# qianyizh/ElasticReconstruction

Measured on AMD Instinct MI355X. Metric: depth frames/sec into 512^3 TSDF (640x480), higher is better.
Workload: dtype f32; 1 GPU; configs[1]; frames_per_gpu=91800, volume_units_touched=122, warp=True, inputs=hbm_resident, parallelism=single GPU

## Files before the change

### elasticreconstruction_amd/_ffi.py

```python
import ctypes as C
import os

_HERE = os.path.dirname(os.path.abspath(__file__))
LIB_PATH = os.environ.get("ER_HIP_LIB") or os.path.join(_HERE, "liber_hip.so")

SYMBOLS = [
    "er_last_error", "er_device_count", "er_abi_version", "er_request_hw_queues", "er_host_alloc", "er_host_free", "er_host_copy_h2d", "er_device_alloc", "er_device_free", "er_device_copy_d2h",
    "er_tsdf_create", "er_tsdf_destroy", "er_tsdf_set_stream", "er_tsdf_synchronize",
    "er_tsdf_wait_event", "er_tsdf_reset", "er_tsdf_status", "er_tsdf_set_unit_shard", "er_unit_owner",
    "er_tsdf_scale_depth", "er_tsdf_reproject", "er_tsdf_integrate", "er_tsdf_integrate_frames", "er_tsdf_prepass_trace", "er_tsdf_set_zbuf_epoch",
    "er_tsdf_unit_count", "er_tsdf_unit_keys", "er_tsdf_read_unit", "er_tsdf_sum_weight",
    "er_tsdf_extract_world", "er_tsdf_extract_surface", "er_tsdf_extract_oriented", "er_tsdf_extract_mesh", "er_mc_table", "er_tsdf_extract_mesh_indexed", "er_mesh_components", "er_tsdf_extract_mesh_cleaned", "er_tsdf_import_world", "er_raycast_params_default", "er_tsdf_raycast", "er_tsdf_raycast_batch", "er_tsdf_export_weighted", "er_tsdf_import_weighted",
    "er_tsdf_export_raw", "er_tsdf_import_raw",
    "er_tsdf_color_enable", "er_tsdf_read_unit_color", "er_tsdf_write_unit_color", "er_tsdf_color_frames", "er_tsdf_reproject_color", "er_tsdf_sample_colors",
    "er_tsdf_band_sizes", "er_tsdf_export_band", "er_tsdf_merge_band", "er_tsdf_import_band", "er_tsdf_drop_units",
    "er_tsdf_set_profiling", "er_tsdf_get_profile", "er_tsdf_set_timeline", "er_tsdf_get_timeline",
    "er_comm_unique_id", "er_comm_create", "er_comm_create_local", "er_comm_create_loopback", "er_comm_destroy", "er_comm_rank", "er_comm_world",
    "er_tsdf_allreduce", "er_comm_merge_stats", "er_comm_merge_stats_owner", "er_frame_block",
    "er_cloud_create", "er_cloud_create_batch", "er_cloud_create_from_tsdf", "er_cloud_destroy", "er_cloud_size",
    "er_icp_count_inliers", "er_icp_align", "er_icp_align_trace", "er_find_correspondence",
    "er_icp_count_inliers_batch", "er_icp_align_batch", "er_find_correspondence_batch", "er_icp_release_workspaces", "er_registration_batch", "er_ransac_fitness_batch", "er_ransac_inliers",
    "er_features_create", "er_features_destroy", "er_features_size", "er_feature_knn", "er_ransac_hypotheses", "er_ransac_params_default", "er_ransac_align", "er_ransac_align_batch",
    "er_odom_params_default", "er_odom_create", "er_odom_destroy", "er_odom_align_pairs", "er_odom_track", "er_frame_to_model_align", "er_frames_to_models_align", "er_odom_linearize", "er_odom_read_maps", "er_odom_tables",
    "er_cloud_read", "er_cloud_voxel_grid", "er_cloud_estimate_normals", "er_fpfh_estimate", "er_features_dim", "er_features_read",
    "er_frag_params_default", "er_frag_create", "er_frag_destroy", "er_frag_lane_bytes", "er_frag_build", "er_frag_count", "er_frag_read",
# ... 72 lines not shown
    L.er_tsdf_create.argtypes = [C.c_int, C.c_int, fp, C.c_int, C.c_int, C.POINTER(vp)]
    L.er_tsdf_destroy.argtypes = [vp]
    L.er_tsdf_set_stream.argtypes = [vp, vp]
    L.er_tsdf_synchronize.argtypes = [vp]
    L.er_tsdf_wait_event.argtypes = [vp, vp]
    L.er_tsdf_reset.argtypes = [vp]
    L.er_tsdf_status.argtypes = [vp, ip, C.POINTER(C.c_long)]
    L.er_tsdf_set_unit_shard.argtypes = [vp, C.c_int, C.c_int]
    L.er_unit_owner.argtypes = [C.c_int, C.c_int]
    L.er_tsdf_scale_depth.argtypes = [vp, vp, vp]
    L.er_tsdf_reproject.argtypes = [vp, vp, vp, C.c_int, C.c_float, vp, vp]
    L.er_tsdf_integrate.argtypes = [vp, vp, vp]
    L.er_tsdf_integrate_frames.argtypes = [vp, C.c_int, vp, C.c_int, vp, C.POINTER(ErWarp)]
    if hasattr(L, "er_tsdf_prepass_trace"):
        L.er_tsdf_prepass_trace.argtypes = [vp, C.c_int, vp, C.c_int, vp, C.POINTER(ErWarp), vp, ip, vp, vp, vp, vp, vp, C.c_int, ip]
    if hasattr(L, "er_tsdf_set_zbuf_epoch"):
        L.er_tsdf_set_zbuf_epoch.argtypes = [vp, C.c_int, C.c_uint]
    L.er_tsdf_unit_count.argtypes = [vp, ip]
    L.er_tsdf_unit_keys.argtypes = [vp, vp]
    L.er_tsdf_read_unit.argtypes = [vp, C.c_int, vp, vp]
    L.er_tsdf_sum_weight.argtypes = [vp, dp]
    L.er_tsdf_extract_world.argtypes = [vp, vp, C.c_long, C.POINTER(C.c_long)]
    L.er_tsdf_extract_surface.argtypes = [vp, vp, C.c_long, C.POINTER(C.c_long)]
    if hasattr(L, "er_tsdf_extract_oriented"):
        L.er_tsdf_extract_oriented.argtypes = [vp, vp, vp, C.c_long, C.POINTER(C.c_long)]
    L.er_tsdf_extract_mesh.argtypes = [vp, vp, C.c_long, C.POINTER(C.c_long)]
    L.er_mc_table.argtypes = [vp]
    if hasattr(L, "er_tsdf_extract_mesh_indexed"):
        L.er_tsdf_extract_mesh_indexed.argtypes = [vp, vp, vp, C.c_long, vp, C.c_long, C.POINTER(C.c_long), C.POINTER(C.c_long)]
        L.er_tsdf_import_world.argtypes = [vp, vp, C.c_long, ip]
# ... 184 lines not shown
```

### elasticreconstruction_amd/csrc/er_tsdf.h

```cpp
#pragma once

#include "er_common.h"
#include "er_tsdf_math.h"

#include "../../include/er_hip.h"

#include <algorithm>
#include <cstdlib>
#include <functional>
#include <utility>
#include <vector>

namespace er_tsdf_k {
using namespace er;

constexpr int kBlock = 256;
constexpr int kEmptyKey = -1;
constexpr uint32_t kZEmpty = 0xFFFFFFFFu;
constexpr uint32_t kZEpochMax = 0xFFFFu;

enum { C_NUNITS = 0, C_NBATCH = 1 , C_POOL_OVERFLOW = 2, C_TABLE_FULL = 3, C_OUT_OF_RANGE = 4,
       C_NBATCH1 = 6, C_NBATCH2 = 7, C_ZERO_WRITE = 8 ,
       C_ZERO_WRITE1 = 10, C_COUNT = 12 };
constexpr int kDepth = 3;
// ... 19 lines not shown
  uint32_t ztag;
};
__global__ void k_reproject_scatter(ReprojArgs A);

constexpr int kFixThreads = 64;
constexpr int kFixBlocks = 256;

constexpr int kScaledPad = 64;
constexpr int kTile = 32;
constexpr int kLoShift = 4;
constexpr int kLoSub = kTile >> kLoShift;
constexpr int kTileKeys = 96;

constexpr int kPrepThreads = 256;
constexpr int kPrepPix = kTile * kTile / kPrepThreads;

template <bool kWide>
__global__ __launch_bounds__(kPrepThreads) void k_prepare(
    const uint16_t* __restrict__ depth, uint32_t* __restrict__ zbuf, int n_frames, int cols, int rows,
    Camera cam, CameraInv cami, const float* __restrict__ lambda, const double* __restrict__ T12, float* __restrict__ scaled,
    int* __restrict__ ht_key, int* __restrict__ ht_slot, unsigned long long* __restrict__ ht_mask, int cap_mask,
    int hash_shift, int* __restrict__ batch, int* __restrict__ nbatch,
    int* __restrict__ counters, float* __restrict__ tile_max, float* __restrict__ tile_lo, float* __restrict__ tile_lo_fine, int2 shard,
    uint32_t* __restrict__ lastzero, uint32_t* __restrict__ zfix, const int* __restrict__ zero_flag, uint32_t ztag);
extern template __global__ void k_prepare<true>(const uint16_t* __restrict__, uint32_t* __restrict__, int, int, int, Camera, CameraInv, const float* __restrict__, const double* __restrict__, float* __restrict__, int* __restrict__, int* __restrict__, unsigned long long* __restrict__, int, int, int* __restrict__, int* __restrict__, int* __restrict__, float* __restrict__, float* __restrict__, float* __restrict__, int2, uint32_t* __restrict__, uint32_t* __restrict__, const int* __restrict__, uint32_t);
extern template __global__ void k_prepare<false>(const uint16_t* __restrict__, uint32_t* __restrict__, int, int, int, Camera, CameraInv, const float* __restrict__, const double* __restrict__, float* __restrict__, int* __restrict__, int* __restrict__, unsigned long long* __restrict__, int, int, int* __restrict__, int* __restrict__, int* __restrict__, float* __restrict__, float* __restrict__, float* __restrict__, int2, uint32_t* __restrict__, uint32_t* __restrict__, const int* __restrict__, uint32_t);

constexpr int kRows = 4;
constexpr int kItemsPerUnit = 256;

// ... 113 lines not shown
```

### elasticreconstruction_amd/csrc/er_tsdf.hip

```cpp
#include "er_tsdf_dev.h"

#include <chrono>
#include <climits>

namespace {

using namespace er_tsdf_k;

constexpr int kNbatchSlot[3] = {C_NBATCH, C_NBATCH1, C_NBATCH2};
constexpr int kZeroFlagSlot[2] = {C_ZERO_WRITE, C_ZERO_WRITE1};

__global__ void k_lambda(float* __restrict__ lambda, int cols, int rows, Camera cam) {
  int p = blockIdx.x * blockDim.x + threadIdx.x;
  if (p >= cols * rows) return;
  lambda[p] = scale_lambda(p % cols, p / cols, cam);
}

__global__ void k_scale_depth(const uint16_t* __restrict__ depth, const float* __restrict__ lambda,
                              float* __restrict__ scaled, int pixels, float itrunc) {
  int p = blockIdx.x * blockDim.x + threadIdx.x;
  if (p >= pixels) return;
  scaled[p] = scale_depth_px(depth[p], lambda[p], itrunc);
}

// ... 356 lines not shown
  ER_HIP_TRY(hipEventRecord(h->consts_done[p], X));
  if (tl && tl_record(h, &tl->ev[1], X)) return 1;
  uint32_t ztag = 0;
  if (warp) {
    if (next_ztag(h, a, h->zbuf[a], (size_t)ER_MAX_BATCH * (size_t)h->pixels, X, &ztag)) return 1;
    const int verts = (warp->resolution + 1) * (warp->resolution + 1) * (warp->resolution + 1);
    const float grid_ul = warp->length / (float)warp->resolution;
    const ReprojArgs RA{depth_dev, n, h->cols, h->rows, h->cam, h->cami, dev_seg, dev_madj, dev_gi, h->ctr, warp->resolution, grid_ul,
                        verts * 3, h->zbuf[a], h->lastzero[a], h->zfix[a], h->counters + kZeroFlagSlot[a], ztag};
    if (launch_reproject(h, RA, n, X)) return 1;
    zsrc = h->zbuf[a];
  }
  if (tl && tl_record(h, &tl->ev[2], X)) return 1;

  const bool wide = h->cols % 4 == 0 && (zsrc || reinterpret_cast<uintptr_t>(depth_dev) % 8 == 0);
  hipLaunchKernelGGL(wide ? k_prepare<true> : k_prepare<false>, dim3((h->cols + kTile - 1) / kTile, (h->rows + kTile - 1) / kTile, n), dim3(kPrepThreads), 0, X,
                     depth_dev, zsrc, n, h->cols, h->rows, h->cam, h->cami, h->lambda, dev_t12, h->scaled[p], h->ht_key, h->ht_slot,
                     h->ht_mask[p], h->ht_cap - 1, h->ht_shift, h->batch[p], nbatch, h->counters,
                     h->tile_max[p], h->tile_lo[p], h->tile_lo_fine[p], make_int2(h->shard_rank, h->shard_world), h->lastzero[a], h->zfix[a],
                     h->counters + kZeroFlagSlot[a], ztag);
  if (tl && tl_record(h, &tl->ev[3], X)) return 1;
  hipLaunchKernelGGL(k_plan, dim3(1), dim3(256), 0, X, h->batch[p], nbatch, h->ht_mask[p], h->ht_key, h->ht_slot, h->unit_key, h->max_units,
                     h->counters, h->plan_rec[p], h->plan[p], warp ? h->counters + kZeroFlagSlot[a] : (int*)nullptr, h->stats);
  ER_HIP_TRY(hipGetLastError());
  if (tl && tl_record(h, &tl->ev[4], X)) return 1;
  ER_HIP_TRY(hipEventRecord(h->pre_done[p], X));

  ER_HIP_TRY(hipStreamWaitEvent(S, h->pre_done[p], 0));
  if (tl && tl_record(h, &tl->ev[5], S)) return 1;
  hipEvent_t e0 = nullptr, e1 = nullptr;
  const bool timed = h->prof_stride > 0 && (h->prof_tick++ % h->prof_stride) == 0;
// ... 258 lines not shown
  hipStream_t C = h->aux_stream[a0];
  if (h->ctr_rd_set[q])
    for (int a = 0; a < kAux; a++)
      if (a != a0) ER_HIP_TRY(hipStreamWaitEvent(C, h->ctr_rd[q][a], 0));
  if (fetch_pinned(h->ctr_dev[q], h->ctr_pinned[q], floats * sizeof(float), C)) return 1;
  ER_HIP_TRY(hipEventRecord(h->ctr_ev[q], C));
  for (int a = 0; a < kAux; a++)
    if (a != a0) ER_HIP_TRY(hipStreamWaitEvent(h->aux_stream[a], h->ctr_ev[q], 0));
  if (also) ER_HIP_TRY(hipStreamWaitEvent(also, h->ctr_ev[q], 0));
  h->ctr = h->ctr_dev[q];
  h->ctr_cur = q;
  return 0;
}

static int launch_reproject(er_tsdf_t h, const ReprojArgs& RA, int n, hipStream_t X) {
  hipLaunchKernelGGL(k_reproject_scatter, dim3((h->cols + 63) / 64, (h->rows + 3) / 4, n), dim3(kBlock), 0, X, RA);
  hipLaunchKernelGGL(k_reproject_fix, dim3(kFixBlocks), dim3(kFixThreads), 0, X, RA);
  ER_HIP_TRY(hipGetLastError());
  return 0;
}

int er_tsdf_reproject(er_tsdf_t h, uint16_t* depth_inout_host, const float* ctr_host, int resolution, float length,
                      const double seg[16], const double madj[16]) {
  if (!h || !depth_inout_host || !ctr_host || !seg || !madj) return er::fail("er_tsdf_reproject: NULL argument");
  if (resolution <= 0) return er::fail("er_tsdf_reproject: bad resolution");
  ER_HIP_TRY(hipSetDevice(h->device));
  const size_t px = (size_t)h->pixels;
  const int verts = (resolution + 1) * (resolution + 1) * (resolution + 1);
  if (sync_all(h)) return 1;
  if (upload_ctr(h, ctr_host, resolution, 1, h->stream)) return 1;
  const int gi = 0;
// ... 94 lines not shown
  ER_HIP_TRY(hipMemcpy(&plan, h->plan[p], sizeof plan, hipMemcpyDeviceToHost));
  if (plan.n_units < 0 || plan.n_units > h->ht_cap) return er::fail("er_tsdf_prepass_trace: the batch lists %d units", plan.n_units);
  if (n_keys) *n_keys = plan.n_units;
  if (keys || masks) {
    std::vector<PlanRec> rec((size_t)plan.n_units);
    if (plan.n_units > 0) ER_HIP_TRY(hipMemcpy(rec.data(), h->plan_rec[p], rec.size() * sizeof(PlanRec), hipMemcpyDeviceToHost));
    std::sort(rec.begin(), rec.end(), [](const PlanRec& a, const PlanRec& b) { return a.key < b.key; });
    for (int i = 0; i < plan.n_units && i < keys_cap; i++) {
      if (keys) keys[i] = rec[(size_t)i].key;
      if (masks) masks[i] = rec[(size_t)i].mask;
    }
  }
  return 0;
}

int er_tsdf_set_zbuf_epoch(er_tsdf_t h, int which, unsigned epoch) {
  if (!h) return er::fail("er_tsdf_set_zbuf_epoch: NULL handle");
  if (which < 0 || which > kZColor) return er::fail("er_tsdf_set_zbuf_epoch: no z-buffer %d (0, 1: the pre-pass streams'; %d: the colour calls')", which, kZColor);
  if (epoch > kZEpochMax) return er::fail("er_tsdf_set_zbuf_epoch: epoch %u above %u", epoch, kZEpochMax);
  ER_HIP_TRY(hipSetDevice(h->device));
  if (sync_all(h)) return 1;
  if (which < kAux && epoch < h->zepoch[which]) {
    ER_HIP_TRY(hipMemsetAsync(h->zbuf[which], 0xFF, (size_t)ER_MAX_BATCH * (size_t)h->pixels * sizeof(uint32_t), h->stream));
    ER_HIP_TRY(hipStreamSynchronize(h->stream));
  }
  h->zepoch[which] = epoch;
  return 0;
}

int er_tsdf_wait_event(er_tsdf_t h, void* hip_event) {
// ... 201 lines not shown
```

### elasticreconstruction_amd/csrc/er_tsdf_dev.h

```cpp
#pragma once

#include "er_tsdf.h"

namespace er_tsdf_k {
namespace {

__device__ __forceinline__ unsigned hash_unit_key(int key, int shift) { return ((unsigned)key * 2654435761u) >> shift; }

__device__ int ht_find_or_insert(int* __restrict__ ht_key, int cap_mask, int shift, int key) {
  unsigned h = hash_unit_key(key, shift);
  for (int probe = 0; probe <= cap_mask; ++probe) {
    int e = (int)((h + (unsigned)probe) & (unsigned)cap_mask);
    int k = __hip_atomic_load(&ht_key[e], __ATOMIC_RELAXED, __HIP_MEMORY_SCOPE_AGENT);
    if (k == key) return e;
    if (k == kEmptyKey) {
      int old = atomicCAS(&ht_key[e], kEmptyKey, key);
      if (old == kEmptyKey || old == key) return e;
    }
  }
  return -1;
}

__device__ __forceinline__ int ht_lookup_slot(const int* __restrict__ ht_key, const int* __restrict__ ht_slot, int cap_mask, int shift, int key) {
  unsigned h = hash_unit_key(key, shift);
// ... 22 lines not shown
}

__device__ __forceinline__ void reproject_scatter_px(const ReprojArgs& A, int f, int u, int v, int replay) {
  const int pixels = A.cols * A.rows;
  const int p = v * A.cols + u;
  const uint16_t d = A.depth[(size_t)f * pixels + p];
  if (d == 0) return;
  int cell;
  uint16_t dd;
  if (!reproject_px(u, v, d, A.cam, A.cami, A.cols, A.rows, A.seg12 + f * 16, A.madj12 + f * 12,
                    A.ctr + (size_t)A.grid_index[f] * A.floats_per_grid, A.res, A.grid_ul, cell, dd))
    return;
  scatter_px(A, f, p, cell, dd, replay);
}

__device__ __forceinline__ uint32_t z_of_epoch(uint32_t z, uint32_t ztag) {
  const uint32_t x = z ^ ztag;
  return x < 0x10000u ? x : kZEmpty;
}

__device__ __forceinline__ uint32_t take_z(uint32_t z, size_t o, uint32_t* __restrict__ lastzero, uint32_t* __restrict__ zfix) {
  if (lastzero[o] == 0) return z;
  const uint32_t r = zfix[o];
  zfix[o] = kZEmpty;
  lastzero[o] = 0;
  return r;
}

}
}
// ... 1 lines not shown
```

### elasticreconstruction_amd/csrc/er_tsdf_math.h

```cpp
#pragma once

#include <math.h>
#include <stdint.h>
#include <string.h>
#include <cmath>

#if defined(__HIPCC__)
#define ER_HD __host__ __device__ __forceinline__
#else
#define ER_HD inline
#endif

namespace er {

struct Camera {
  float fx, fy, cx, cy, icp_trunc, integration_trunc;
};

struct CameraInv {
  double inv_fx, inv_fy;
  int pp_small;
  int pad;
};

// ... 43 lines not shown
  int xi = ((int)v0 + 256 * 64) / 64;
  int yi = ((int)v1 + 256 * 64) / 64;
  int zi = ((int)v2 + 256 * 64) / 64;
  return xi * 512 * 512 + yi * 512 + zi;
}

ER_HD int touch_key_exact(int u, int v, uint16_t d, const Camera& c, const double* T) {
  double x, y, z;
  uvd2xyz(u, v, d, c, x, y, z);
  double p0 = ((T[0] * x + T[1] * y) + T[2] * z) + T[3];
  double p1 = ((T[4] * x + T[5] * y) + T[6] * z) + T[7];
  double p2 = ((T[8] * x + T[9] * y) + T[10] * z) + T[11];
  return key_from_voxels(floor(p0 / kUnitLength + 0.5), floor(p1 / kUnitLength + 0.5), floor(p2 / kUnitLength + 0.5));
}

ER_HD int touch_key(int u, int v, uint16_t d, const Camera& c, const CameraInv& ci, const double* T) {
  const double z = (double)d * 0.001;
  const double xr = (double)((float)u - c.cx) * ci.inv_fx;
  const double yr = (double)((float)v - c.cy) * ci.inv_fy;
  const double k = (512.0 / 3.0) / 64.0, k0 = 0.5 / 64.0 + 256.0;
  const double w0 = fma(fma(z, fma(T[0], xr, fma(T[1], yr, T[2])), T[3]), k, k0);
  const double w1 = fma(fma(z, fma(T[4], xr, fma(T[5], yr, T[6])), T[7]), k, k0);
  const double w2 = fma(fma(z, fma(T[8], xr, fma(T[9], yr, T[10])), T[11]), k, k0);
  const double f0 = floor(w0), f1 = floor(w1), f2 = floor(w2);
  const double m = 0.5 - 1.5e-8;
  const bool safe = (fabs((w0 - f0) - 0.5) < m) & (fabs((w1 - f1) - 0.5) < m) & (fabs((w2 - f2) - 0.5) < m);
  if (safe) {
    if (!((fabs(w0 - 256.0) < 256.0) & (fabs(w1 - 256.0) < 256.0) & (fabs(w2 - 256.0) < 256.0))) return -1;
    return ((int)f0 << 18) | ((int)f1 << 9) | (int)f2;
  }
  return touch_key_exact(u, v, d, c, T);
}

ER_HD int unit_owner(int key, int world) {
  const int xi = key >> 18, yi = (key >> 9) & 511, zi = key & 511;
  return (xi + yi + zi) % world;
}

ER_HD float unit_shift(int idx) { return (float)((double)((idx - 256) * 64) * kUnitLength); }

ER_HD float grid_coord(int i, float shift) { return (float)((double)i * kUnitLength + (double)shift); }

ER_HD void div2_inrange(float n0, float n1, float d, float& q0, float& q1) {
#if defined(__HIP_DEVICE_COMPILE__)
  float r = __builtin_amdgcn_rcpf(d);
  r = fmaf(fmaf(-d, r, 1.0f), r, r);
// ... 243 lines not shown
                            int cols, int rows, const float* __restrict__ tile_max, int tiles_x, int tiles_y, bool* inside) {
  return patch_may_update_box(g0, g0, g1lo, g1hi, g2lo, g2hi, f, c, cols, rows, tile_max, tiles_x, tiles_y, inside);
}

ER_HD double fast_rcp64(double x) {
#if defined(__HIP_DEVICE_COMPILE__)
  double r = __builtin_amdgcn_rcp(x);
  r = fma(fma(-x, r, 1.0), r, r);
  r = fma(fma(-x, r, 1.0), r, r);
  return r;
#else
  return 1.0 / x;
#endif
}

ER_HD void cube_coords(int u, int v, uint16_t d, const Camera& c, const CameraInv& ci, const double* seg, float out[3]) {
  const double z = (double)d * 0.001;
  const double xr = (double)((float)u - c.cx) * ci.inv_fx;
  const double yr = (double)((float)v - c.cy) * ci.inv_fy;
  bool safe = true;
  for (int r = 0; r < 3; r++) {
    const double q = fma(z, fma(seg[4 * r], xr, fma(seg[4 * r + 1], yr, seg[4 * r + 2])), seg[4 * r + 3]);
    const double delta = seg[12 + r];
    const float lo = (float)(q - delta), hi = (float)(q + delta);
    safe = safe & (lo == hi);
    out[r] = lo;
  }
  if (safe) return;
  double xe, ye, ze;
  uvd2xyz(u, v, d, c, xe, ye, ze);
  for (int r = 0; r < 3; r++) out[r] = (float)(((seg[4 * r] * xe + seg[4 * r + 1] * ye) + seg[4 * r + 2] * ze) + seg[4 * r + 3]);
}

inline void cube_coord_deltas(const double* seg, const Camera& c, int cols, int rows, double out3[3]) {
  const double zmax = 65.535;
  const double xa = fmax(fabs(0.0 - (double)c.cx), fabs((double)(cols - 1) - (double)c.cx)) * zmax / (double)c.fx;
  const double ya = fmax(fabs(0.0 - (double)c.cy), fabs((double)(rows - 1) - (double)c.cy)) * zmax / (double)c.fy;
  for (int r = 0; r < 3; r++)
    out3[r] = 4e-15 * (fabs(seg[4 * r]) * xa + fabs(seg[4 * r + 1]) * ya + fabs(seg[4 * r + 2]) * zmax + fabs(seg[4 * r + 3]));
}

ER_HD double round_pixel(double e, double f, double e2, double rcp_e2, double cc, bool cc_small) {
  const double w = fma(e * f, rcp_e2, cc + 0.5);
  const double fl = floor(w), fr = w - fl;
  if (cc_small && fabs(w) < 1e6 && fr > 1e-6 && fr < 1.0 - 1e-6) return fl;
  return floor((e * f / e2 + cc) + 0.5);
}

ER_HD unsigned lattice_stride(const float*) { return 12u; }
ER_HD void lattice_vertex(const float* __restrict__ ctr, unsigned byte_off, float v[3]) {
  const float* p = reinterpret_cast<const float*>(reinterpret_cast<const char*>(ctr) + byte_off);
  v[0] = p[0]; v[1] = p[1]; v[2] = p[2];
}

template <typename Lattice>
ER_HD bool reproject_px(int u, int v, uint16_t d, const Camera& c, const CameraInv& ci, int cols, int rows, const double* seg,
                        const double* madj, const Lattice* __restrict__ ctr, int res, float grid_ul, int& cell, uint16_t& dd,
                        double* e_out = nullptr) {
  float pt[3];
  cube_coords(u, v, d, c, ci, seg, pt);
  float a0, a1, a2;
  if ((grid_ul >= 0x1p-30f) & (grid_ul <= 0x1p30f)) {
    div3_inrange(pt[0], pt[1], pt[2], grid_ul, a0, a1, a2);
  } else {
    a0 = pt[0] / grid_ul;
    a1 = pt[1] / grid_ul;
    a2 = pt[2] / grid_ul;
  }
  float f0 = floorf(a0), f1 = floorf(a1), f2 = floorf(a2);
  float fres = (float)res;
  if (!(f0 >= 0.0f && f0 < fres && f1 >= 0.0f && f1 < fres && f2 >= 0.0f && f2 < fres)) return false;
  int c0 = (int)f0, c1 = (int)f1, c2 = (int)f2;
  float r0 = a0 - f0, r1 = a1 - f1, r2 = a2 - f2;
  int n1 = res + 1, n2 = n1 * n1;
  const unsigned vs = lattice_stride(ctr);
// ... 43 lines not shown
  double e2 = ((madj[8] * pa + madj[9] * pb) + madj[10] * pc) + madj[11];
  if (e_out) { e_out[0] = e0; e_out[1] = e1; e_out[2] = e2; }
  if (!(e2 > 0.0)) return false;
  const double re = fast_rcp64(e2);
  double uu = round_pixel(e0, (double)c.fx, e2, re, (double)c.cx, ci.pp_small);
  double vv = round_pixel(e1, (double)c.fy, e2, re, (double)c.cy, ci.pp_small);
  const double ulim = cols < 640 ? (double)cols : 640.0, vlim = rows < 480 ? (double)rows : 480.0;
  if (!(uu >= 0.0 && uu < ulim && vv >= 0.0 && vv < vlim)) return false;
  double dz = floor(e2 * 1000.0 + 0.5);
  if (!(dz < 2147483648.0)) return false;
  dd = (uint16_t)((uint32_t)(int)dz & 0xFFFFu);
  cell = (int)vv * cols + (int)uu;
  return true;
}


}
```

### elasticreconstruction_amd/csrc/er_tsdf_pre.hip

```cpp
#include "er_tsdf_dev.h"

namespace er_tsdf_k {

__global__ void k_reproject_scatter(ReprojArgs A) {
  const int f = blockIdx.z;
  const int u = blockIdx.x * 64 + (threadIdx.x & 63);
  const int v = blockIdx.y * 4 + (threadIdx.x >> 6);
  if (u >= A.cols || v >= A.rows) return;
  reproject_scatter_px(A, f, u, v, 0);
}

namespace {

__device__ void touch_unit(int key, int f, int* __restrict__ ht_key, int* __restrict__ ht_slot,
                           unsigned long long* __restrict__ ht_mask, int cap_mask, int hash_shift,
                           int* __restrict__ batch, int* __restrict__ nbatch, int* __restrict__ counters, int2 shard) {
  if (shard.y > 1 && unit_owner(key, shard.y) != shard.x) return;
  const int e = ht_find_or_insert(ht_key, cap_mask, hash_shift, key);
  if (e < 0) {
    atomicOr(&counters[C_TABLE_FULL], 1);
    return;
  }
  const unsigned long long bit = 1ull << f;
  const unsigned long long seen = __hip_atomic_load(&ht_mask[e], __ATOMIC_RELAXED, __HIP_MEMORY_SCOPE_AGENT);
// ... 57 lines not shown
static_assert(kTile == 32 && kPrepPix == 4 && kPrepThreads == 256, "k_prepare: 8 column groups x 32 rows of 4 pixels; a wave is 8 rows of the tile");
static_assert(kLoShift == 4 && kLoSub == 2, "k_prepare: a sub-tile is 4 threads (one quad) wide and 2 waves high; lane bit 2 is its column");
constexpr int kPrepCols = kTile / kPrepPix;
constexpr int kPrepWaveRows = 64 / kPrepCols;
constexpr int kPrepSubWaves = (1 << kLoShift) / kPrepWaveRows;

template <bool kWide>
__global__ __launch_bounds__(kPrepThreads) void k_prepare(
    const uint16_t* __restrict__ depth, uint32_t* __restrict__ zbuf, int n_frames, int cols, int rows,
    Camera cam, CameraInv cami, const float* __restrict__ lambda, const double* __restrict__ T12, float* __restrict__ scaled,
    int* __restrict__ ht_key, int* __restrict__ ht_slot, unsigned long long* __restrict__ ht_mask, int cap_mask,
    int hash_shift, int* __restrict__ batch, int* __restrict__ nbatch,
    int* __restrict__ counters, float* __restrict__ tile_max, float* __restrict__ tile_lo, float* __restrict__ tile_lo_fine, int2 shard,
    uint32_t* __restrict__ lastzero, uint32_t* __restrict__ zfix, const int* __restrict__ zero_flag, uint32_t ztag) {
  __shared__ int s_keys[kTileKeys];
  __shared__ int s_n;
  __shared__ float s_wmax[kPrepThreads / 64], s_wlo[kLoSub][kLoSub][kPrepSubWaves];
  const int pixels = cols * rows;
  const int f = blockIdx.z;
  const bool replayed = zbuf && ((zero_flag[f >> 5] >> (f & 31)) & 1);
  const int c = threadIdx.x & (kPrepCols - 1), r = threadIdx.x / kPrepCols;
  const int x0 = blockIdx.x * kTile + c * kPrepPix, y = blockIdx.y * kTile + r;
  if (threadIdx.x == 0) s_n = 0;
  __syncthreads();
  const int p = y * cols + x0;
  const size_t o = (size_t)f * pixels + p;
  float* __restrict__ const sc_out = scaled + ((size_t)f * (pixels + kScaledPad) + p);
  uint16_t d[kPrepPix];
  float lam[kPrepPix];
  bool in[kPrepPix];
#pragma unroll
  for (int j = 0; j < kPrepPix; j++) {
    d[j] = 0;
    lam[j] = 0.0f;
    in[j] = y < rows && x0 + (kWide ? 0 : j) < cols;
  }
  if constexpr (kWide) {
    if (in[0]) {
      if (zbuf) {
        const uint4 zv = *reinterpret_cast<const uint4*>(zbuf + o);
        uint32_t z[kPrepPix] = {z_of_epoch(zv.x, ztag), z_of_epoch(zv.y, ztag), z_of_epoch(zv.z, ztag), z_of_epoch(zv.w, ztag)};
        if (replayed) {
#pragma unroll
          for (int j = 0; j < kPrepPix; j++) z[j] = take_z(z[j], o + j, lastzero, zfix);
        }
#pragma unroll
        for (int j = 0; j < kPrepPix; j++) d[j] = (z[j] == kZEmpty) ? (uint16_t)0 : (uint16_t)z[j];
      } else {
        uint2 dv;
        __builtin_memcpy(&dv, __builtin_assume_aligned(depth + o, 8), 8);
        d[0] = (uint16_t)dv.x;
        d[1] = (uint16_t)(dv.x >> 16);
        d[2] = (uint16_t)dv.y;
        d[3] = (uint16_t)(dv.y >> 16);
      }
      const float4 lv = *reinterpret_cast<const float4*>(lambda + p);
      lam[0] = lv.x;
      lam[1] = lv.y;
      lam[2] = lv.z;
      lam[3] = lv.w;
    }
  } else {
#pragma unroll
    for (int j = 0; j < kPrepPix; j++) {
      if (in[j]) {
        if (zbuf) {
          uint32_t z = z_of_epoch(zbuf[o + j], ztag);
          if (replayed) z = take_z(z, o + j, lastzero, zfix);
          d[j] = (z == kZEmpty) ? (uint16_t)0 : (uint16_t)z;
        } else {
          d[j] = depth[o + j];
        }
        lam[j] = lambda[p + j];
      }
    }
  }
  float wmax = 0.0f, vlo = 3.0e38f, sc[kPrepPix];
  int key[kPrepPix];
#pragma unroll
  for (int j = 0; j < kPrepPix; j++) {
    key[j] = -1;
    sc[j] = 0.0f;
    if (in[j]) {
      sc[j] = scale_depth_px(d[j], lam[j], cam.integration_trunc);
      if constexpr (!kWide) sc_out[j] = sc[j];
      wmax = fmaxf(wmax, sc[j]);
      vlo = fminf(vlo, sc[j] > 0.001f ? sc[j] : 0.0f);
      if (d[j] > 0) {
        key[j] = touch_key(x0 + j, y, d[j], cam, cami, T12 + f * 12);
        if (key[j] < 0) atomicAdd(&counters[C_OUT_OF_RANGE], 1);
      }
    }
  }
  if constexpr (kWide) {
    if (in[0]) *reinterpret_cast<float4*>(sc_out) = make_float4(sc[0], sc[1], sc[2], sc[3]);
  }
  const int left = dpp_mov<kDppRowShr1>(key[kPrepPix - 1]);
#pragma unroll
  for (int j = 0; j < kPrepPix; j++) {
    const bool leader = key[j] >= 0 && (j == 0 ? (c == 0 || left != key[0]) : key[j - 1] != key[j]);
    if (leader) {
      const int slot = atomicAdd(&s_n, 1);
      if (slot < kTileKeys) {
        s_keys[slot] = key[j];
      } else {
        touch_unit(key[j], f, ht_key, ht_slot, ht_mask, cap_mask, hash_shift, batch, nbatch, counters, shard);
      }
    }
  }
  const int lane = threadIdx.x & 63, wave = threadIdx.x >> 6;
  wmax = reduce_wave(wmax, FMax());
  vlo = reduce_half_columns(vlo, FMin());
  if (lane == 0) s_wmax[wave] = wmax;
  if ((lane & ~4) == 0) s_wlo[wave / kPrepSubWaves][lane >> 2][wave % kPrepSubWaves] = vlo;
  __syncthreads();
  if (threadIdx.x == 0) {
    float m = 0.0f, lo = 3.0e38f;
    for (int w = 0; w < kPrepThreads / 64; w++) m = fmaxf(m, s_wmax[w]);
    for (int e = 0; e < kLoSub * kLoSub * kPrepSubWaves; e++) lo = fminf(lo, (&s_wlo[0][0][0])[e]);
    const size_t t = ((size_t)blockIdx.y * gridDim.x + blockIdx.x) * ER_MAX_BATCH + f;
    tile_max[t] = m;
    tile_lo[t] = lo;
  }
  if ((int)threadIdx.x < kLoSub * kLoSub) {
    const int sr = threadIdx.x / kLoSub, sg = threadIdx.x % kLoSub;
    float lo = 3.0e38f;
    for (int w = 0; w < kPrepSubWaves; w++) lo = fminf(lo, s_wlo[sr][sg][w]);
    const int lx = blockIdx.x * kLoSub + sg, ly = blockIdx.y * kLoSub + sr;
    const int lo_tx = (cols + (1 << kLoShift) - 1) >> kLoShift, lo_ty = (rows + (1 << kLoShift) - 1) >> kLoShift;
    if (lx < lo_tx && ly < lo_ty) tile_lo_fine[((size_t)ly * lo_tx + lx) * ER_MAX_BATCH + f] = lo;
  }
  const int n = min(s_n, kTileKeys);
  if ((int)threadIdx.x < n) {
    const int k = s_keys[threadIdx.x];
    bool dup = false;
    for (int j = 0; j < (int)threadIdx.x; j++) dup = dup || (s_keys[j] == k);
    if (!dup) touch_unit(k, f, ht_key, ht_slot, ht_mask, cap_mask, hash_shift, batch, nbatch, counters, shard);
  }
}

#define ER_PREPARE_INST(W) \
  template __global__ void k_prepare<W>(const uint16_t* __restrict__, uint32_t* __restrict__, int, int, int, Camera, CameraInv, const float* __restrict__, \
                                        const double* __restrict__, float* __restrict__, int* __restrict__, int* __restrict__,                             \
                                        unsigned long long* __restrict__, int, int, int* __restrict__, int* __restrict__, int* __restrict__,               \
                                        float* __restrict__, float* __restrict__, float* __restrict__, int2, uint32_t* __restrict__,                       \
                                        uint32_t* __restrict__, const int* __restrict__, uint32_t);
ER_PREPARE_INST(true)
ER_PREPARE_INST(false)
#undef ER_PREPARE_INST

}
```

### include/er_hip.h

```cpp
#ifndef ER_HIP_H_
#define ER_HIP_H_

#include <stddef.h>
#include <stdint.h>

#ifdef __cplusplus
extern "C" {
#endif

#define ER_UNIT_RES 64
#define ER_UNIT_VOX (64 * 64 * 64)
#define ER_MAX_BATCH 64

const char* er_last_error(void);
int er_device_count(void);
int er_abi_version(void);
int er_request_hw_queues(int n);

void* er_host_alloc(size_t bytes);
int er_host_free(void* p);
int er_host_copy_h2d(void* dev_dst, const void* host_src, size_t bytes);
void* er_device_alloc(size_t bytes, int device);
int er_device_free(void* p);
int er_device_copy_d2h(void* host_dst, const void* dev_src, size_t bytes);
// ... 17 lines not shown
int er_tsdf_synchronize(er_tsdf_t h);

int er_tsdf_scale_depth(er_tsdf_t h, const uint16_t* depth_host, float* scaled_host);

int er_tsdf_reproject(er_tsdf_t h, uint16_t* depth_inout_host, const float* ctr_host, int resolution, float length,
                      const double seg[16], const double madj[16]);

int er_tsdf_integrate(er_tsdf_t h, const uint16_t* depth_host, const double T[16]);

int er_tsdf_integrate_frames(er_tsdf_t h, int n, const uint16_t* depth, int depth_on_device, const double* T,
                             const er_warp* warp);

int er_tsdf_prepass_trace(er_tsdf_t h, int n, const uint16_t* depth, int depth_on_device, const double* T, const er_warp* warp,
                          float* scaled, int* scaled_pad, float* tile_max, float* tile_lo, float* tile_lo_fine,
                          int* keys, unsigned long long* masks, int keys_cap, int* n_keys);

int er_tsdf_set_zbuf_epoch(er_tsdf_t h, int which, unsigned epoch);

int er_tsdf_wait_event(er_tsdf_t h, void* hip_event);

int er_tsdf_reset(er_tsdf_t h);

#define ER_STATUS_POOL_EXHAUSTED 1
#define ER_STATUS_TABLE_FULL 2
int er_tsdf_status(er_tsdf_t h, int* flags, long* out_of_range_pixels);

int er_tsdf_unit_count(er_tsdf_t h, int* count);
int er_tsdf_unit_keys(er_tsdf_t h, int* keys_host);
int er_tsdf_read_unit(er_tsdf_t h, int key, float* sdf_host, float* weight_host);

// ... 289 lines not shown
```

Before: 201,300 frames/s.

## Process several frames per block in prepare and reproject-scatter kernels

The prepare and reproject-scatter kernels now loop over a chunk of frames per block (ER_PRE_CHUNK, default 5) instead of one frame per grid z-slice. Per-pixel ray terms are computed once and reused across the chunk, and the next frame's depth is prefetched. Inline-asm barriers pin camera parameters to scalar registers. This cuts grid size and redundant per-pixel setup, but leaves fewer blocks in flight and serialises frames within a block, with double-buffered shared counters and extra syncs per frame.

After: 200,000 frames/s. No clear change (-0.7%).

```diff
diff --git a/elasticreconstruction_amd/_ffi.py b/elasticreconstruction_amd/_ffi.py
--- a/elasticreconstruction_amd/_ffi.py
+++ b/elasticreconstruction_amd/_ffi.py
@@ -8,7 +8,7 @@
     "er_last_error", "er_device_count", "er_abi_version", "er_request_hw_queues", "er_host_alloc", "er_host_free", "er_host_copy_h2d", "er_device_alloc", "er_device_free", "er_device_copy_d2h",
     "er_tsdf_create", "er_tsdf_destroy", "er_tsdf_set_stream", "er_tsdf_synchronize",
     "er_tsdf_wait_event", "er_tsdf_reset", "er_tsdf_status", "er_tsdf_set_unit_shard", "er_unit_owner",
-    "er_tsdf_scale_depth", "er_tsdf_reproject", "er_tsdf_integrate", "er_tsdf_integrate_frames", "er_tsdf_prepass_trace", "er_tsdf_set_zbuf_epoch",
+    "er_tsdf_scale_depth", "er_tsdf_reproject", "er_tsdf_integrate", "er_tsdf_integrate_frames", "er_tsdf_prepass_trace", "er_tsdf_prepass_chunk", "er_tsdf_set_zbuf_epoch",
     "er_tsdf_unit_count", "er_tsdf_unit_keys", "er_tsdf_read_unit", "er_tsdf_sum_weight",
     "er_tsdf_extract_world", "er_tsdf_extract_surface", "er_tsdf_extract_oriented", "er_tsdf_extract_mesh", "er_mc_table", "er_tsdf_extract_mesh_indexed", "er_mesh_components", "er_tsdf_extract_mesh_cleaned", "er_tsdf_import_world", "er_raycast_params_default", "er_tsdf_raycast", "er_tsdf_raycast_batch", "er_tsdf_export_weighted", "er_tsdf_import_weighted",
     "er_tsdf_export_raw", "er_tsdf_import_raw",
@@ -111,6 +111,8 @@
     L.er_tsdf_integrate_frames.argtypes = [vp, C.c_int, vp, C.c_int, vp, C.POINTER(ErWarp)]
     if hasattr(L, "er_tsdf_prepass_trace"):
         L.er_tsdf_prepass_trace.argtypes = [vp, C.c_int, vp, C.c_int, vp, C.POINTER(ErWarp), vp, ip, vp, vp, vp, vp, vp, C.c_int, ip]
+    if hasattr(L, "er_tsdf_prepass_chunk"):
+        L.er_tsdf_prepass_chunk.argtypes = []
     if hasattr(L, "er_tsdf_set_zbuf_epoch"):
         L.er_tsdf_set_zbuf_epoch.argtypes = [vp, C.c_int, C.c_uint]
     L.er_tsdf_unit_count.argtypes = [vp, ip]
diff --git a/elasticreconstruction_amd/csrc/er_tsdf.h b/elasticreconstruction_amd/csrc/er_tsdf.h
--- a/elasticreconstruction_amd/csrc/er_tsdf.h
+++ b/elasticreconstruction_amd/csrc/er_tsdf.h
@@ -57,6 +57,11 @@
 
 constexpr int kPrepThreads = 256;
 constexpr int kPrepPix = kTile * kTile / kPrepThreads;
+#ifndef ER_PRE_CHUNK
+#define ER_PRE_CHUNK 5
+#endif
+constexpr int kPreChunk = ER_PRE_CHUNK;
+static_assert(kPreChunk >= 1 && kPreChunk <= ER_MAX_BATCH, "a chunk is at least a frame and at most a batch");
 
 template <bool kWide>
 __global__ __launch_bounds__(kPrepThreads) void k_prepare(
diff --git a/elasticreconstruction_amd/csrc/er_tsdf.hip b/elasticreconstruction_amd/csrc/er_tsdf.hip
--- a/elasticreconstruction_amd/csrc/er_tsdf.hip
+++ b/elasticreconstruction_amd/csrc/er_tsdf.hip
@@ -394,7 +394,8 @@
   if (tl && tl_record(h, &tl->ev[2], X)) return 1;
 
   const bool wide = h->cols % 4 == 0 && (zsrc || reinterpret_cast<uintptr_t>(depth_dev) % 8 == 0);
-  hipLaunchKernelGGL(wide ? k_prepare<true> : k_prepare<false>, dim3((h->cols + kTile - 1) / kTile, (h->rows + kTile - 1) / kTile, n), dim3(kPrepThreads), 0, X,
+  hipLaunchKernelGGL(wide ? k_prepare<true> : k_prepare<false>, dim3((h->cols + kTile - 1) / kTile, (h->rows + kTile - 1) / kTile, (n + kPreChunk - 1) / kPreChunk),
+                     dim3(kPrepThreads), 0, X,
                      depth_dev, zsrc, n, h->cols, h->rows, h->cam, h->cami, h->lambda, dev_t12, h->scaled[p], h->ht_key, h->ht_slot,
                      h->ht_mask[p], h->ht_cap - 1, h->ht_shift, h->batch[p], nbatch, h->counters,
                      h->tile_max[p], h->tile_lo[p], h->tile_lo_fine[p], make_int2(h->shard_rank, h->shard_world), h->lastzero[a], h->zfix[a],
@@ -683,7 +684,8 @@
 }
 
 static int launch_reproject(er_tsdf_t h, const ReprojArgs& RA, int n, hipStream_t X) {
-  hipLaunchKernelGGL(k_reproject_scatter, dim3((h->cols + 63) / 64, (h->rows + 3) / 4, n), dim3(kBlock), 0, X, RA);
+  if (n != RA.n_frames) return er::fail("launch_reproject: %d frames, arguments for %d", n, RA.n_frames);
+  hipLaunchKernelGGL(k_reproject_scatter, dim3((h->cols + 63) / 64, (h->rows + 3) / 4, (n + kPreChunk - 1) / kPreChunk), dim3(kBlock), 0, X, RA);
   hipLaunchKernelGGL(k_reproject_fix, dim3(kFixBlocks), dim3(kFixThreads), 0, X, RA);
   ER_HIP_TRY(hipGetLastError());
   return 0;
@@ -808,6 +810,8 @@
   return 0;
 }
 
+int er_tsdf_prepass_chunk(void) { return kPreChunk; }
+
 int er_tsdf_set_zbuf_epoch(er_tsdf_t h, int which, unsigned epoch) {
   if (!h) return er::fail("er_tsdf_set_zbuf_epoch: NULL handle");
   if (which < 0 || which > kZColor) return er::fail("er_tsdf_set_zbuf_epoch: no z-buffer %d (0, 1: the pre-pass streams'; %d: the colour calls')", which, kZColor);
diff --git a/elasticreconstruction_amd/csrc/er_tsdf_dev.h b/elasticreconstruction_amd/csrc/er_tsdf_dev.h
--- a/elasticreconstruction_amd/csrc/er_tsdf_dev.h
+++ b/elasticreconstruction_amd/csrc/er_tsdf_dev.h
@@ -60,6 +60,17 @@
   scatter_px(A, f, p, cell, dd, replay);
 }
 
+__device__ __forceinline__ void per_frame(float& x) { asm volatile("" : "+s"(x)); }
+__device__ __forceinline__ void per_frame(int& x) { asm volatile("" : "+s"(x)); }
+__device__ __forceinline__ void per_frame_lane(int& x) { asm volatile("" : "+v"(x)); }
+__device__ __forceinline__ void per_frame(Camera& c) {
+  per_frame(c.fx);
+  per_frame(c.fy);
+  per_frame(c.cx);
+  per_frame(c.cy);
+  per_frame(c.integration_trunc);
+}
+
 __device__ __forceinline__ uint32_t z_of_epoch(uint32_t z, uint32_t ztag) {
   const uint32_t x = z ^ ztag;
   return x < 0x10000u ? x : kZEmpty;
diff --git a/elasticreconstruction_amd/csrc/er_tsdf_math.h b/elasticreconstruction_amd/csrc/er_tsdf_math.h
--- a/elasticreconstruction_amd/csrc/er_tsdf_math.h
+++ b/elasticreconstruction_amd/csrc/er_tsdf_math.h
@@ -81,10 +81,13 @@
   return key_from_voxels(floor(p0 / kUnitLength + 0.5), floor(p1 / kUnitLength + 0.5), floor(p2 / kUnitLength + 0.5));
 }
 
-ER_HD int touch_key(int u, int v, uint16_t d, const Camera& c, const CameraInv& ci, const double* T) {
+ER_HD void ray_terms(int u, int v, const Camera& c, const CameraInv& ci, double& xr, double& yr) {
+  xr = (double)((float)u - c.cx) * ci.inv_fx;
+  yr = (double)((float)v - c.cy) * ci.inv_fy;
+}
+
+ER_HD int touch_key(int u, int v, uint16_t d, double xr, double yr, const Camera& c, const double* T) {
   const double z = (double)d * 0.001;
-  const double xr = (double)((float)u - c.cx) * ci.inv_fx;
-  const double yr = (double)((float)v - c.cy) * ci.inv_fy;
   const double k = (512.0 / 3.0) / 64.0, k0 = 0.5 / 64.0 + 256.0;
   const double w0 = fma(fma(z, fma(T[0], xr, fma(T[1], yr, T[2])), T[3]), k, k0);
   const double w1 = fma(fma(z, fma(T[4], xr, fma(T[5], yr, T[6])), T[7]), k, k0);
@@ -97,6 +100,12 @@
     return ((int)f0 << 18) | ((int)f1 << 9) | (int)f2;
   }
   return touch_key_exact(u, v, d, c, T);
+}
+
+ER_HD int touch_key(int u, int v, uint16_t d, const Camera& c, const CameraInv& ci, const double* T) {
+  double xr, yr;
+  ray_terms(u, v, c, ci, xr, yr);
+  return touch_key(u, v, d, xr, yr, c, T);
 }
 
 ER_HD int unit_owner(int key, int world) {
@@ -370,10 +379,8 @@
 #endif
 }
 
-ER_HD void cube_coords(int u, int v, uint16_t d, const Camera& c, const CameraInv& ci, const double* seg, float out[3]) {
+ER_HD void cube_coords(int u, int v, uint16_t d, double xr, double yr, const Camera& c, const double* seg, float out[3]) {
   const double z = (double)d * 0.001;
-  const double xr = (double)((float)u - c.cx) * ci.inv_fx;
-  const double yr = (double)((float)v - c.cy) * ci.inv_fy;
   bool safe = true;
   for (int r = 0; r < 3; r++) {
     const double q = fma(z, fma(seg[4 * r], xr, fma(seg[4 * r + 1], yr, seg[4 * r + 2])), seg[4 * r + 3]);
@@ -388,6 +395,12 @@
   for (int r = 0; r < 3; r++) out[r] = (float)(((seg[4 * r] * xe + seg[4 * r + 1] * ye) + seg[4 * r + 2] * ze) + seg[4 * r + 3]);
 }
 
+ER_HD void cube_coords(int u, int v, uint16_t d, const Camera& c, const CameraInv& ci, const double* seg, float out[3]) {
+  double xr, yr;
+  ray_terms(u, v, c, ci, xr, yr);
+  cube_coords(u, v, d, xr, yr, c, seg, out);
+}
+
 inline void cube_coord_deltas(const double* seg, const Camera& c, int cols, int rows, double out3[3]) {
   const double zmax = 65.535;
   const double xa = fmax(fabs(0.0 - (double)c.cx), fabs((double)(cols - 1) - (double)c.cx)) * zmax / (double)c.fx;
@@ -410,11 +423,11 @@
 }
 
 template <typename Lattice>
-ER_HD bool reproject_px(int u, int v, uint16_t d, const Camera& c, const CameraInv& ci, int cols, int rows, const double* seg,
-                        const double* madj, const Lattice* __restrict__ ctr, int res, float grid_ul, int& cell, uint16_t& dd,
-                        double* e_out = nullptr) {
+ER_HD bool reproject_px(int u, int v, uint16_t d, double xr, double yr, const Camera& c, const CameraInv& ci, int cols, int rows,
+                        const double* seg, const double* madj, const Lattice* __restrict__ ctr, int res, float grid_ul, int& cell,
+                        uint16_t& dd, double* e_out = nullptr) {
   float pt[3];
-  cube_coords(u, v, d, c, ci, seg, pt);
+  cube_coords(u, v, d, xr, yr, c, seg, pt);
   float a0, a1, a2;
   if ((grid_ul >= 0x1p-30f) & (grid_ul <= 0x1p30f)) {
     div3_inrange(pt[0], pt[1], pt[2], grid_ul, a0, a1, a2);
@@ -488,5 +501,14 @@
   return true;
 }
 
-
-}
+template <typename Lattice>
+ER_HD bool reproject_px(int u, int v, uint16_t d, const Camera& c, const CameraInv& ci, int cols, int rows, const double* seg,
+                        const double* madj, const Lattice* __restrict__ ctr, int res, float grid_ul, int& cell, uint16_t& dd,
+                        double* e_out = nullptr) {
+  double xr, yr;
+  ray_terms(u, v, c, ci, xr, yr);
+  return reproject_px(u, v, d, xr, yr, c, ci, cols, rows, seg, madj, ctr, res, grid_ul, cell, dd, e_out);
+}
+
+
+}
diff --git a/elasticreconstruction_amd/csrc/er_tsdf_pre.hip b/elasticreconstruction_amd/csrc/er_tsdf_pre.hip
--- a/elasticreconstruction_amd/csrc/er_tsdf_pre.hip
+++ b/elasticreconstruction_amd/csrc/er_tsdf_pre.hip
@@ -2,12 +2,53 @@
 
 namespace er_tsdf_k {
 
+namespace {
+
+__device__ __forceinline__ void scatter_frames(int u, int v, int f0, int f1, const uint16_t* __restrict__ depth, int cols_, int rows_, Camera cam_,
+                                               CameraInv cami, const double* __restrict__ seg12, const double* __restrict__ madj12,
+                                               const int* __restrict__ grid_index, const float* __restrict__ ctr, int res_, float grid_ul_,
+                                               int floats_per_grid, uint32_t* __restrict__ zbuf, uint32_t* __restrict__ lastzero,
+                                               int* __restrict__ zero_flag, uint32_t ztag) {
+  const ReprojArgs A{depth, f1, cols_, rows_, cam_, cami, seg12, madj12, grid_index, ctr, res_, grid_ul_, floats_per_grid, zbuf, lastzero, nullptr, zero_flag, ztag};
+  const int pixels = cols_ * rows_;
+  const int p = v * cols_ + u;
+  double xr, yr;
+  ray_terms(u, v, cam_, cami, xr, yr);
+  const uint16_t* src = depth + ((size_t)f0 * pixels + p);
+  int d = *src;
+  asm volatile("" : "+v"(d));
+#pragma unroll 1
+  for (int f = f0; f < f1; f++) {
+    src += pixels;
+    const int d_next = (f + 1 < f1) ? *src : 0;
+    Camera cam = cam_;
+    int cols = cols_, rows = rows_, res = res_;
+    float grid_ul = grid_ul_;
+    per_frame(cam);
+    per_frame(cols);
+    per_frame(rows);
+    per_frame(res);
+    per_frame(grid_ul);
+    int cell = 0;
+    uint16_t dd = 0;
+    const bool hit = d != 0 &&
+                     reproject_px(u, v, (uint16_t)d, xr, yr, cam, cami, cols, rows, seg12 + f * 16, madj12 + f * 12,
+                                  ctr + (size_t)grid_index[f] * floats_per_grid, res, grid_ul, cell, dd);
+    d = d_next;
+    asm volatile("" : "+v"(d));
+    if (hit) scatter_px(A, f, p, cell, dd, 0);
+  }
+}
+
+}
+
 __global__ void k_reproject_scatter(ReprojArgs A) {
-  const int f = blockIdx.z;
   const int u = blockIdx.x * 64 + (threadIdx.x & 63);
   const int v = blockIdx.y * 4 + (threadIdx.x >> 6);
   if (u >= A.cols || v >= A.rows) return;
-  reproject_scatter_px(A, f, u, v, 0);
+  const int f0 = blockIdx.z * kPreChunk, f1 = min(f0 + kPreChunk, A.n_frames);
+  scatter_frames(u, v, f0, f1, A.depth, A.cols, A.rows, A.cam, A.cami, A.seg12, A.madj12, A.grid_index, A.ctr, A.res, A.grid_ul, A.floats_per_grid,
+                 A.zbuf, A.lastzero, A.zero_flag, A.ztag);
 }
 
 namespace {
@@ -95,128 +136,150 @@
     int* __restrict__ counters, float* __restrict__ tile_max, float* __restrict__ tile_lo, float* __restrict__ tile_lo_fine, int2 shard,
     uint32_t* __restrict__ lastzero, uint32_t* __restrict__ zfix, const int* __restrict__ zero_flag, uint32_t ztag) {
   __shared__ int s_keys[kTileKeys];
-  __shared__ int s_n;
+  __shared__ int s_n[2];
   __shared__ float s_wmax[kPrepThreads / 64], s_wlo[kLoSub][kLoSub][kPrepSubWaves];
   const int pixels = cols * rows;
-  const int f = blockIdx.z;
-  const bool replayed = zbuf && ((zero_flag[f >> 5] >> (f & 31)) & 1);
-  const int c = threadIdx.x & (kPrepCols - 1), r = threadIdx.x / kPrepCols;
-  const int x0 = blockIdx.x * kTile + c * kPrepPix, y = blockIdx.y * kTile + r;
-  if (threadIdx.x == 0) s_n = 0;
-  __syncthreads();
-  const int p = y * cols + x0;
-  const size_t o = (size_t)f * pixels + p;
-  float* __restrict__ const sc_out = scaled + ((size_t)f * (pixels + kScaledPad) + p);
-  uint16_t d[kPrepPix];
-  float lam[kPrepPix];
+  const int f0 = blockIdx.z * kPreChunk, f1 = min(f0 + kPreChunk, n_frames);
+  int p0;
   bool in[kPrepPix];
-#pragma unroll
-  for (int j = 0; j < kPrepPix; j++) {
-    d[j] = 0;
-    lam[j] = 0.0f;
-    in[j] = y < rows && x0 + (kWide ? 0 : j) < cols;
-  }
-  if constexpr (kWide) {
-    if (in[0]) {
-      if (zbuf) {
-        const uint4 zv = *reinterpret_cast<const uint4*>(zbuf + o);
-        uint32_t z[kPrepPix] = {z_of_epoch(zv.x, ztag), z_of_epoch(zv.y, ztag), z_of_epoch(zv.z, ztag), z_of_epoch(zv.w, ztag)};
-        if (replayed) {
-#pragma unroll
-          for (int j = 0; j < kPrepPix; j++) z[j] = take_z(z[j], o + j, lastzero, zfix);
-        }
-#pragma unroll
-        for (int j = 0; j < kPrepPix; j++) d[j] = (z[j] == kZEmpty) ? (uint16_t)0 : (uint16_t)z[j];
-      } else {
-        uint2 dv;
-        __builtin_memcpy(&dv, __builtin_assume_aligned(depth + o, 8), 8);
-        d[0] = (uint16_t)dv.x;
-        d[1] = (uint16_t)(dv.x >> 16);
-        d[2] = (uint16_t)dv.y;
-        d[3] = (uint16_t)(dv.y >> 16);
-      }
-      const float4 lv = *reinterpret_cast<const float4*>(lambda + p);
-      lam[0] = lv.x;
-      lam[1] = lv.y;
-      lam[2] = lv.z;
-      lam[3] = lv.w;
-    }
-  } else {
-#pragma unroll
-    for (int j = 0; j < kPrepPix; j++) {
+  double xr[kPrepPix], yr;
+  {
+    const int c = threadIdx.x & (kPrepCols - 1), r = threadIdx.x / kPrepCols;
+    const int x0 = blockIdx.x * kTile + c * kPrepPix, y = blockIdx.y * kTile + r;
+    p0 = y * cols + x0;
+#pragma unroll
+    for (int j = 0; j < kPrepPix; j++) {
+      in[j] = y < rows && x0 + (kWide ? 0 : j) < cols;
+      ray_terms(x0 + j, y, cam, cami, xr[j], yr);
+    }
+  }
+  const size_t t_out = ((size_t)blockIdx.y * gridDim.x + blockIdx.x) * ER_MAX_BATCH;
+#pragma unroll 1
+  for (int f = f0; f < f1; f++) {
+    int& s_nf = s_n[(f - f0) & 1];
+    const bool replayed = zbuf && ((zero_flag[f >> 5] >> (f & 31)) & 1);
+    int tid = threadIdx.x, p = p0;
+    per_frame_lane(tid);
+    per_frame_lane(p);
+    const int c = tid & (kPrepCols - 1), r = tid / kPrepCols;
+    const int x0 = blockIdx.x * kTile + c * kPrepPix, y = blockIdx.y * kTile + r;
+    Camera camf = cam;
+    per_frame(camf);
+    int2 shardf = shard;
+    per_frame(shardf.x);
+    per_frame(shardf.y);
+    if (tid == 0) s_nf = 0;
+    __syncthreads();
+    const size_t o = (size_t)f * pixels + p;
+    float* __restrict__ const sc_out = scaled + ((size_t)f * (pixels + kScaledPad) + p);
+    uint16_t d[kPrepPix];
+    float lam[kPrepPix];
+#pragma unroll
+    for (int j = 0; j < kPrepPix; j++) {
+      d[j] = 0;
+      lam[j] = 0.0f;
+    }
+    if constexpr (kWide) {
+      if (in[0]) {
+        if (zbuf) {
+          const uint4 zv = *reinterpret_cast<const uint4*>(zbuf + o);
+          uint32_t z[kPrepPix] = {z_of_epoch(zv.x, ztag), z_of_epoch(zv.y, ztag), z_of_epoch(zv.z, ztag), z_of_epoch(zv.w, ztag)};
+          if (replayed) {
+#pragma unroll
+            for (int j = 0; j < kPrepPix; j++) z[j] = take_z(z[j], o + j, lastzero, zfix);
+          }
+#pragma unroll
+          for (int j = 0; j < kPrepPix; j++) d[j] = (z[j] == kZEmpty) ? (uint16_t)0 : (uint16_t)z[j];
+        } else {
+          uint2 dv;
+          __builtin_memcpy(&dv, __builtin_assume_aligned(depth + o, 8), 8);
+          d[0] = (uint16_t)dv.x;
+          d[1] = (uint16_t)(dv.x >> 16);
+          d[2] = (uint16_t)dv.y;
+          d[3] = (uint16_t)(dv.y >> 16);
+        }
+        const float4 lv = *reinterpret_cast<const float4*>(lambda + p);
+        lam[0] = lv.x;
+        lam[1] = lv.y;
+        lam[2] = lv.z;
+        lam[3] = lv.w;
+      }
+    } else {
+#pragma unroll
+      for (int j = 0; j < kPrepPix; j++) {
+        if (in[j]) {
+          if (zbuf) {
+            uint32_t z = z_of_epoch(zbuf[o + j], ztag);
+            if (replayed) z = take_z(z, o + j, lastzero, zfix);
+            d[j] = (z == kZEmpty) ? (uint16_t)0 : (uint16_t)z;
+          } else {
+            d[j] = depth[o + j];
+          }
+          lam[j] = lambda[p + j];
+        }
+      }
+    }
+    float wmax = 0.0f, vlo = 3.0e38f, sc[kPrepPix];
+    int key[kPrepPix];
+#pragma unroll
+    for (int j = 0; j < kPrepPix; j++) {
+      key[j] = -1;
+      sc[j] = 0.0f;
       if (in[j]) {
-        if (zbuf) {
-          uint32_t z = z_of_epoch(zbuf[o + j], ztag);
-          if (replayed) z = take_z(z, o + j, lastzero, zfix);
-          d[j] = (z == kZEmpty) ? (uint16_t)0 : (uint16_t)z;
+        sc[j] = scale_depth_px(d[j], lam[j], camf.integration_trunc);
+        if constexpr (!kWide) sc_out[j] = sc[j];
+        wmax = fmaxf(wmax, sc[j]);
+        vlo = fminf(vlo, sc[j] > 0.001f ? sc[j] : 0.0f);
+        if (d[j] > 0) {
+          key[j] = touch_key(x0 + j, y, d[j], xr[j], yr, camf, T12 + f * 12);
+          if (key[j] < 0) atomicAdd(&counters[C_OUT_OF_RANGE], 1);
+        }
+      }
+    }
+    if constexpr (kWide) {
+      if (in[0]) *reinterpret_cast<float4*>(sc_out) = make_float4(sc[0], sc[1], sc[2], sc[3]);
+    }
+    const int left = dpp_mov<kDppRowShr1>(key[kPrepPix - 1]);
+#pragma unroll
+    for (int j = 0; j < kPrepPix; j++) {
+      const bool leader = key[j] >= 0 && (j == 0 ? (c == 0 || left != key[0]) : key[j - 1] != key[j]);
+      if (leader) {
+        const int slot = atomicAdd(&s_nf, 1);
+        if (slot < kTileKeys) {
+          s_keys[slot] = key[j];
         } else {
-          d[j] = depth[o + j];
-        }
-        lam[j] = lambda[p + j];
-      }
-    }
-  }
-  float wmax = 0.0f, vlo = 3.0e38f, sc[kPrepPix];
-  int key[kPrepPix];
-#pragma unroll
-  for (int j = 0; j < kPrepPix; j++) {
-    key[j] = -1;
-    sc[j] = 0.0f;
-    if (in[j]) {
-      sc[j] = scale_depth_px(d[j], lam[j], cam.integration_trunc);
-      if constexpr (!kWide) sc_out[j] = sc[j];
-      wmax = fmaxf(wmax, sc[j]);
-      vlo = fminf(vlo, sc[j] > 0.001f ? sc[j] : 0.0f);
-      if (d[j] > 0) {
-        key[j] = touch_key(x0 + j, y, d[j], cam, cami, T12 + f * 12);
-        if (key[j] < 0) atomicAdd(&counters[C_OUT_OF_RANGE], 1);
-      }
-    }
-  }
-  if constexpr (kWide) {
-    if (in[0]) *reinterpret_cast<float4*>(sc_out) = make_float4(sc[0], sc[1], sc[2], sc[3]);
-  }
-  const int left = dpp_mov<kDppRowShr1>(key[kPrepPix - 1]);
-#pragma unroll
-  for (int j = 0; j < kPrepPix; j++) {
-    const bool leader = key[j] >= 0 && (j == 0 ? (c == 0 || left != key[0]) : key[j - 1] != key[j]);
-    if (leader) {
-      const int slot = atomicAdd(&s_n, 1);
-      if (slot < kTileKeys) {
-        s_keys[slot] = key[j];
-      } else {
-        touch_unit(key[j], f, ht_key, ht_slot, ht_mask, cap_mask, hash_shift, batch, nbatch, counters, shard);
-      }
-    }
-  }
-  const int lane = threadIdx.x & 63, wave = threadIdx.x >> 6;
-  wmax = reduce_wave(wmax, FMax());
-  vlo = reduce_half_columns(vlo, FMin());
-  if (lane == 0) s_wmax[wave] = wmax;
-  if ((lane & ~4) == 0) s_wlo[wave / kPrepSubWaves][lane >> 2][wave % kPrepSubWaves] = vlo;
-  __syncthreads();
-  if (threadIdx.x == 0) {
-    float m = 0.0f, lo = 3.0e38f;
-    for (int w = 0; w < kPrepThreads / 64; w++) m = fmaxf(m, s_wmax[w]);
-    for (int e = 0; e < kLoSub * kLoSub * kPrepSubWaves; e++) lo = fminf(lo, (&s_wlo[0][0][0])[e]);
-    const size_t t = ((size_t)blockIdx.y * gridDim.x + blockIdx.x) * ER_MAX_BATCH + f;
-    tile_max[t] = m;
-    tile_lo[t] = lo;
-  }
-  if ((int)threadIdx.x < kLoSub * kLoSub) {
-    const int sr = threadIdx.x / kLoSub, sg = threadIdx.x % kLoSub;
-    float lo = 3.0e38f;
-    for (int w = 0; w < kPrepSubWaves; w++) lo = fminf(lo, s_wlo[sr][sg][w]);
-    const int lx = blockIdx.x * kLoSub + sg, ly = blockIdx.y * kLoSub + sr;
-    const int lo_tx = (cols + (1 << kLoShift) - 1) >> kLoShift, lo_ty = (rows + (1 << kLoShift) - 1) >> kLoShift;
-    if (lx < lo_tx && ly < lo_ty) tile_lo_fine[((size_t)ly * lo_tx + lx) * ER_MAX_BATCH + f] = lo;
-  }
-  const int n = min(s_n, kTileKeys);
-  if ((int)threadIdx.x < n) {
-    const int k = s_keys[threadIdx.x];
-    bool dup = false;
-    for (int j = 0; j < (int)threadIdx.x; j++) dup = dup || (s_keys[j] == k);
-    if (!dup) touch_unit(k, f, ht_key, ht_slot, ht_mask, cap_mask, hash_shift, batch, nbatch, counters, shard);
+          touch_unit(key[j], f, ht_key, ht_slot, ht_mask, cap_mask, hash_shift, batch, nbatch, counters, shardf);
+        }
+      }
+    }
+    const int lane = tid & 63, wave = tid >> 6;
+    wmax = reduce_wave(wmax, FMax());
+    vlo = reduce_half_columns(vlo, FMin());
+    if (lane == 0) s_wmax[wave] = wmax;
+    if ((lane & ~4) == 0) s_wlo[wave / kPrepSubWaves][lane >> 2][wave % kPrepSubWaves] = vlo;
+    __syncthreads();
+    if (tid == 0) {
+      float m = 0.0f, lo = 3.0e38f;
+      for (int w = 0; w < kPrepThreads / 64; w++) m = fmaxf(m, s_wmax[w]);
+      for (int e = 0; e < kLoSub * kLoSub * kPrepSubWaves; e++) lo = fminf(lo, (&s_wlo[0][0][0])[e]);
+      tile_max[t_out + f] = m;
+      tile_lo[t_out + f] = lo;
+    }
+    if (tid < kLoSub * kLoSub) {
+      const int sr = tid / kLoSub, sg = tid % kLoSub;
+      float lo = 3.0e38f;
+      for (int w = 0; w < kPrepSubWaves; w++) lo = fminf(lo, s_wlo[sr][sg][w]);
+      const int lx = blockIdx.x * kLoSub + sg, ly = blockIdx.y * kLoSub + sr;
+      const int lo_tx = (cols + (1 << kLoShift) - 1) >> kLoShift, lo_ty = (rows + (1 << kLoShift) - 1) >> kLoShift;
+      if (lx < lo_tx && ly < lo_ty) tile_lo_fine[((size_t)ly * lo_tx + lx) * ER_MAX_BATCH + f] = lo;
+    }
+    const int n = min(s_nf, kTileKeys);
+    if (tid < n) {
+      const int k = s_keys[tid];
+      bool dup = false;
+      for (int j = 0; j < tid; j++) dup = dup || (s_keys[j] == k);
+      if (!dup) touch_unit(k, f, ht_key, ht_slot, ht_mask, cap_mask, hash_shift, batch, nbatch, counters, shardf);
+    }
   }
 }
 
diff --git a/include/er_hip.h b/include/er_hip.h
--- a/include/er_hip.h
+++ b/include/er_hip.h
@@ -55,6 +55,8 @@
 int er_tsdf_prepass_trace(er_tsdf_t h, int n, const uint16_t* depth, int depth_on_device, const double* T, const er_warp* warp,
                           float* scaled, int* scaled_pad, float* tile_max, float* tile_lo, float* tile_lo_fine,
                           int* keys, unsigned long long* masks, int keys_cap, int* n_keys);
+
+int er_tsdf_prepass_chunk(void);
 
 int er_tsdf_set_zbuf_epoch(er_tsdf_t h, int which, unsigned epoch);
 
```
